# meharkhurana03/cm3d

Hardware: AMD Instinct MI355X
Metric: pseudo-label frames/sec on nuScenes-shaped sweeps (higher is better)
Workload: dtype f32; 1 GPU; c2: 256 frames/GPU x (35000x1 pts, 6 cams, 20 masks 1600x900), masks resident as rle; frames_per_gpu=256, points_per_frame=35000, masks_per_frame=20, lane_points=50000, mask_input=rle, batches_in_flight=4, distinct_batches=4, cloud_materialised=False

## Files before the change

### cm3d_amd/csrc/medoid.hip

```cpp
#include "common.h"
#include "worklist.h"
#include <stdlib.h>

#ifndef MD_WAVES
#define MD_WAVES 4
#endif
#define MD_THREADS (MD_WAVES * 64)
#ifndef MD_STAGE
#define MD_STAGE 256
#endif

#ifndef MD_LONG_MIN
#define MD_LONG_MIN 256
#endif
#ifndef MD_BATCH_LONG
#define MD_BATCH_LONG 448
#endif
#define MD_LONG_MAX 100000
static __device__ __forceinline__ bool md_two_pass(int M) { return M > MD_LONG_MIN && M < MD_LONG_MAX; }
static_assert(MD_BATCH_LONG >= MD_LONG_MIN && MD_BATCH_LONG <= CM3D_MEDOID_TILE * MD_UNI && MD_BATCH_LONG % CM3D_MEDOID_TILE == 0,
              "the batch limit is a boundary between two of the one-count classes");
static __device__ __forceinline__ bool md_batch_long(const TileDesc *desc, int ntiles) { return ntiles > 0 && __builtin_amdgcn_readfirstlane(desc[0].M) > MD_BATCH_LONG; }

#ifndef MD_APPROX_MFMA
// ... 243 lines not shown

template <typename Fetch>
static __device__ __forceinline__ void md_approx_tile(Fetch fetch, float *s_rows, int off, int M, int jt, float *__restrict__ approx_out)
{
    const int lane = cm3d_lane();
    float qx = 0.f, qy = 0.f, qz = 0.f;
    {
        const int j = jt * 64 + lane;
        const float4 q = fetch(off + min(j, M - 1));
        if (j < M) { qx = q.x; qy = q.y; qz = q.z; }
    }
    float4 g4[MDA_STAGE / 64];
#pragma unroll
    for (int c = 0; c < MDA_STAGE / 64; ++c) g4[c] = fetch(off + min(c * 64 + lane, M - 1));
    const float qn = (qx * qx + qy * qy) + qz * qz;
    const bool cols_ok = !__ballot(!mda_point_ok(qx, qy, qz, qn));
    const float bx = qx * MDA_S, by = qy * MDA_S, bz = qz * MDA_S, bn = qn * MDA_S2;
    f2 s = {0.f, 0.f};
    bool scaled = false;
    for (int i0 = 0; i0 < M; i0 += MDA_STAGE) {
        __builtin_amdgcn_wave_barrier();
        float4 rr[MDA_STAGE / 64];
        bool rows_ok = true;
#pragma unroll
        for (int c = 0; c < MDA_STAGE / 64; ++c) {
            rr[c] = make_float4(0.f, 0.f, 0.f, 0.f);
            if (i0 + c * 64 + lane < M) {
                const float4 p = g4[c];
                rr[c] = make_float4(-2.0f * p.x, -2.0f * p.y, -2.0f * p.z, (p.x * p.x + p.y * p.y) + p.z * p.z);
                rows_ok &= mda_point_ok(p.x, p.y, p.z, rr[c].w);
            }
        }
#pragma unroll
        for (int c = 0; c < MDA_STAGE / 64; ++c) g4[c] = fetch(off + min(i0 + MDA_STAGE + c * 64 + lane, M - 1));
        const bool scaled_now = MD_SCALED_ROUTES && cols_ok && !__ballot(!rows_ok);
#pragma unroll
        for (int c = 0; c < MDA_STAGE / 64; ++c) {
            float4 r = rr[c];
            if (scaled_now) r = make_float4(r.x * MDA_S, r.y * MDA_S, r.z * MDA_S, r.w * MDA_S2);
            *reinterpret_cast<float4 *>(s_rows + 4 * (c * 64 + lane)) = r;
        }
        scaled = scaled_now;
        __builtin_amdgcn_fence(__ATOMIC_RELEASE, "wavefront");
        __builtin_amdgcn_wave_barrier();
        __builtin_amdgcn_fence(__ATOMIC_ACQUIRE, "wavefront");
        const int cnt = min(MDA_STAGE, M - i0), full = cnt & ~31;
        const float a5 = full + (lane & 31) < cnt ? 1.0f : 0.0f;
        if (scaled) {
            for (int r0 = 0; r0 < full; r0 += 32) s = md_approx_step<true>(s_rows, r0, 1.0f, bx, by, bz, bn, s);
            if (cnt & 31) s = md_approx_step<true>(s_rows, full, a5, bx, by, bz, bn, s);
        } else {
            const float ux = bx * 65536.0f, uy = by * 65536.0f, uz = bz * 65536.0f, un = bn * 4294967296.0f;
            for (int r0 = 0; r0 < full; r0 += 32) s = md_approx_step<false>(s_rows, r0, 1.0f, ux, uy, uz, un, s);
            if (cnt & 31) s = md_approx_step<false>(s_rows, full, a5, ux, uy, uz, un, s);
        }
    }
    const float t0 = (s.x + __shfl_xor(s.x, 32, 64)) * 65536.0f, t1 = (s.y + __shfl_xor(s.y, 32, 64)) * 65536.0f;
    if (lane < 32) {
        const int j = jt * 64 + lane;
        if (j < M) approx_out[off + j] = t0;
        if (j + 32 < M) approx_out[off + j + 32] = t1;
    }
}

#ifndef MD_INW_MAX
#define MD_INW_MAX MD_STAGE
#endif
#ifndef MD_INW_GC
#define MD_INW_GC 2
#endif
static_assert(MD_INW_MAX <= MD_STAGE && MD_INW_GC % 2 == 0 && MD_INW_GC * 64 * sizeof(float) <= 64 * sizeof(float4),
              "a round's terms fit the storage of its 64 staged rows");

static __device__ __forceinline__ f2 md_exact_dist2s(float m2x, float m2y, float m2z, float n, float4 qa, float4 qb)
{
    f2 acc = (f2){m2x, m2x} * (f2){qa.x, qb.x};
    acc = PK_FMA(((f2){m2y, m2y}), ((f2){qa.y, qb.y}), acc);
    acc = PK_FMA(((f2){m2z, m2z}), ((f2){qa.z, qb.z}), acc);
    acc = acc + (f2){n, n};
    acc = md_pk_add_clamp01(acc, (f2){qa.w, qb.w});
    return md_sqrt_core2z(acc);
}

static __device__ __forceinline__ bool md_inwave_tile(float4 *s_row, int cnt, int M, int jt, bool act, float qx, float qy, float qz, float qn,
                                                      float &bs, int &bj)
{
    const int lane = cm3d_lane();
    const float a = md_rows<false, true, true, true>(s_row, cnt, qx, qy, qz, qn, 0.0f) * 65536.0f;
    const float rel = 1.05f * (float)(M + 2) * 1.1920928955078125e-07f, abs_e = (float)M * 2.1e-14f;
    const float e = fmaf(a, rel, abs_e);
    const float thr = cm3d_wave_reduce_t(act ? a + e : INFINITY, [](float x, float y) { return fminf(x, y); });
    const bool all = __ballot(act && !(a < INFINITY)) != 0;
    const uint64_t cm = __ballot(act && (all || !(a - e > thr)));
    const int C = (int)__popcll(cm);
    if (C < 1 || C > MD_INW_GC) return false;
    float4 q[MD_INW_GC];
    int myj = 0x7FFFFFFF;
    {
        uint64_t rest = cm;
        const int first = __builtin_ctzll(cm);
#pragma unroll
        for (int c = 0; c < MD_INW_GC; ++c) {
            const int cl = rest ? __builtin_ctzll(rest) : first;
            if (rest && lane == c) myj = jt * 64 + cl;
            rest &= rest - 1;
            q[c] = make_float4(__int_as_float(__builtin_amdgcn_readlane(__float_as_int(qx), cl)), __int_as_float(__builtin_amdgcn_readlane(__float_as_int(qy), cl)),
                               __int_as_float(__builtin_amdgcn_readlane(__float_as_int(qz), cl)), __int_as_float(__builtin_amdgcn_readlane(__float_as_int(qn), cl)));
        }
    }
    float s = 0.0f;
    for (int r0 = 0; r0 < M; r0 += 64) {
        const bool valid = r0 + lane < M;
        const int row = min(r0 + lane, cnt - 1);
        const float *f = reinterpret_cast<const float *>(s_row) + (row >> 1) * 8 + (row & 1);
        const float m2x = f[0], m2y = f[2], m2z = f[4], n = f[6];
        float *t = reinterpret_cast<float *>(s_row + r0);
        __builtin_amdgcn_fence(__ATOMIC_RELEASE, "wavefront");
        __builtin_amdgcn_wave_barrier();
        __builtin_amdgcn_fence(__ATOMIC_ACQUIRE, "wavefront");
#pragma unroll
        for (int c = 0; c < MD_INW_GC; c += 2) {
            if (c < C) {
                const f2 d = md_exact_dist2s(m2x, m2y, m2z, n, q[c], q[c + 1]);
                t[c * 64 + lane] = valid ? d.x : 0.0f;
                t[(c + 1) * 64 + lane] = valid ? d.y : 0.0f;
            }
        }
        __builtin_amdgcn_fence(__ATOMIC_RELEASE, "wavefront");
        __builtin_amdgcn_wave_barrier();
        __builtin_amdgcn_fence(__ATOMIC_ACQUIRE, "wavefront");
        if (lane < C) {
            const float4 *tr = reinterpret_cast<const float4 *>(t + lane * 64);
            const int n16 = (min(64, M - r0) + 15) >> 4;
            for (int k0 = 0; k0 < n16; ++k0) {
                float4 v[4];
#pragma unroll
                for (int k = 0; k < 4; ++k) v[k] = tr[4 * k0 + k];
#pragma unroll
                for (int k = 0; k < 4; ++k) { s = s + v[k].x; s = s + v[k].y; s = s + v[k].z; s = s + v[k].w; }
            }
        }
    }
    bs = lane < C ? s * 65536.0f : INFINITY;
    bj = myj;
    return true;
}

template <bool WITH_LONG, bool INDEXED>
__global__ __launch_bounds__(MD_THREADS, 4) void k_medoid_tiles(const float4 *__restrict__ points,
                                                              const int32_t *__restrict__ pt_off,
                                                              const int32_t *__restrict__ mask_frame, int n_masks,
                                                              const int32_t *__restrict__ tile_off,
                                                              const int32_t *__restrict__ hit_row,
                                                              const TileDesc *__restrict__ desc,
                                                              TileBest *__restrict__ tile_best, int tile_cap,
                                                              float *__restrict__ colsum_opt, float *__restrict__ approx_opt,
                                                              int32_t *__restrict__ long_list, int32_t *__restrict__ feedback)
{
    __shared__ float4 s_row_all[MD_WAVES][MD_STAGE];
    if (!WITH_LONG && blockIdx.x == 0 && threadIdx.x == 0) {
        long_list[0] = 0;
        if (feedback) feedback[0] = md_batch_long(desc, min(tile_off[n_masks], tile_cap)) ? 1 : 0;
    }
    const int wave = threadIdx.x >> 6, lane = cm3d_lane();
    float4 *s_row = s_row_all[wave];
    const int ntiles = min(tile_off[n_masks], tile_cap);
    if (ntiles <= 0) return;
    if ((approx_opt != nullptr && md_batch_long(desc, ntiles)) != WITH_LONG) return;
    for (int t = blockIdx.x * MD_WAVES + wave; t < ntiles; t += gridDim.x * MD_WAVES) {
        const TileDesc d = desc[t];
        const int off = __builtin_amdgcn_readfirstlane(d.off), M = __builtin_amdgcn_readfirstlane(d.M);
        const int jt = __builtin_amdgcn_readfirstlane(d.jt);
        const float4 *P = INDEXED ? points + pt_off[mask_frame[__builtin_amdgcn_readfirstlane(d.m)]] : points;
        auto fetch = [&](int q) { return INDEXED ? P[hit_row[q]] : P[q]; };
        const int j = jt * 64 + lane;
        const bool act = j < M;
        float qx = 0.f, qy = 0.f, qz = 0.f, qn = 0.f;
        {
            const float4 q = fetch(off + min(j, M - 1));
            if (act) {
                qx = q.x; qy = q.y; qz = q.z;
                qn = (q.x * q.x + q.y * q.y) + q.z * q.z;
            }
        }
        float s = 0.f;
        const bool col_safe = !__ballot(act && !md_col_safe(qn));
        const bool col_scal = !__ballot(act && !mda_point_ok(qx, qy, qz, qn));
        const bool direct = M <= 25;
        const bool inw_ok = !WITH_LONG && colsum_opt == nullptr && !direct && M <= MD_INW_MAX;
        bool inw = false;
        float bs_inw = INFINITY;
        int bj_inw = 0x7FFFFFFF;
        const bool approx = WITH_LONG && md_two_pass(M);
        if (WITH_LONG && approx && MD_APPROX_MFMA) {
            md_approx_tile(fetch, reinterpret_cast<float *>(s_row), off, M, jt, approx_opt);
            continue;
        }
        for (int i0 = 0; i0 < M; i0 += MD_STAGE) {
            __builtin_amdgcn_wave_barrier();
            float4 g[MD_STAGE / 64];
            bool rows_safe = true, rows_scal = true;
#pragma unroll
            for (int c = 0; c < MD_STAGE / 64; ++c)
                g[c] = fetch(off + min(i0 + c * 64 + lane, M - 1));
#pragma unroll
            for (int c = 0; c < MD_STAGE / 64; ++c) {
                if (i0 + c * 64 + lane < M) {
                    float4 r = g[c];
                    r.w = (r.x * r.x + r.y * r.y) + r.z * r.z;
                    rows_safe &= md_row_safe(r.w);
                    rows_scal &= mda_point_ok(r.x, r.y, r.z, r.w);
                    if (!direct) { r.x = -2.0f * r.x; r.y = -2.0f * r.y; r.z = -2.0f * r.z; }
                    g[c] = r;
                }
            }
            const bool scaled = MD_SCALED_ROUTES && !direct && !approx && col_scal && !__ballot(!rows_scal);
#pragma unroll
            for (int c = 0; c < MD_STAGE / 64; ++c) {
                if (i0 + c * 64 + lane < M) {
                    float4 r = g[c];
                    if (scaled) r = make_float4(r.x * MDA_S, r.y * MDA_S, r.z * MDA_S, r.w * MDA_S2);
                    md_stage(s_row, c * 64 + lane, r);
                }
            }
            int cnt = min(MD_STAGE, M - i0);
            if (!direct) {
                const int pad = (8 - (cnt & 7)) & 7;
                if (lane < pad) md_stage(s_row, cnt + lane, make_float4(0.0f, 0.0f, 0.0f, -INFINITY));
                cnt += pad;
            }
            __builtin_amdgcn_fence(__ATOMIC_RELEASE, "wavefront");
            __builtin_amdgcn_wave_barrier();
            __builtin_amdgcn_fence(__ATOMIC_ACQUIRE, "wavefront");
            const bool safe = col_safe && !__ballot(!rows_safe);
            if (scaled && inw_ok && safe && md_inwave_tile(s_row, cnt, M, jt, act, qx * MDA_S, qy * MDA_S, qz * MDA_S, qn * MDA_S2, bs_inw, bj_inw))
                inw = true;
            else if (scaled)
                s = md_rows<false, false, true, true>(s_row, cnt, qx * MDA_S, qy * MDA_S, qz * MDA_S, qn * MDA_S2, s * MDA_S) * 65536.0f;
            else
                s = direct ? md_rows<true>(s_row, cnt, qx, qy, qz, qn, s)
                           : (approx ? md_rows<false, true>(s_row, cnt, qx, qy, qz, qn, s)
                                     : (safe ? md_rows<false, false, true>(s_row, cnt, qx, qy, qz, qn, s)
                                             : (WITH_LONG ? md_rows<false>(s_row, cnt, qx, qy, qz, qn, s) : md_rows_plain(s_row, min(MD_STAGE, M - i0), qx, qy, qz, qn, s))));
        }
        if (approx) {
            if (act) approx_opt[off + j] = s;
            continue;
        }
        if (act && colsum_opt) colsum_opt[off + j] = s;
        float bs = inw ? bs_inw : (act ? s : INFINITY);
        int bj = inw ? bj_inw : (act ? j : 0x7FFFFFFF);
        auto better = [](float s1, int j1, float s2, int j2) {
            const bool n1 = s1 != s1, n2 = s2 != s2;
            if (n1 != n2) return n1;
            if (!n1 && s1 != s2) return s1 < s2;
            return j1 < j2;
        };
        {
            const Cm3dValIdx red = cm3d_wave_reduce_t(Cm3dValIdx{bs, bj}, [&](Cm3dValIdx a_, Cm3dValIdx b_) { return better(b_.s, b_.j, a_.s, a_.j) ? b_ : a_; });
            bs = red.s; bj = red.j;
        }
        if (lane == 0) { tile_best[d.t].s = bs; tile_best[d.t].j = bj; }
    }
}

__global__ __launch_bounds__(256) void k_medoid_reduce(const float4 *__restrict__ points, const int32_t *__restrict__ pt_off,
                                                       const int32_t *__restrict__ mask_frame, int n_masks,
                                                       const int32_t *__restrict__ hit_off,
                                                       const int32_t *__restrict__ tile_off,
                                                       const int32_t *__restrict__ hit_row, int idx_cap,
                                                       const TileBest *__restrict__ tile_best, int tile_cap, int two_pass,
                                                       const TileDesc *__restrict__ desc, int32_t *__restrict__ long_list,
                                                       int32_t *__restrict__ medoid_pos, float *__restrict__ centroid)
{
    const int m = blockIdx.x * blockDim.x + threadIdx.x;
    const bool is_long = two_pass && md_batch_long(desc, min(tile_off[n_masks], tile_cap)) && m < n_masks && md_two_pass(hit_off[m + 1] - hit_off[m]);
    {
        const uint64_t lm = __ballot(is_long);
        if (lm) {
            int base = 0;
            if (cm3d_lane() == 0) base = atomicAdd(&long_list[0], (int)__popcll(lm));
            base = __builtin_amdgcn_readfirstlane(base);
            if (is_long) long_list[1 + base + cm3d_mbcnt(lm)] = m;
        }
    }
    if (m >= n_masks || is_long) return;
    const int t0 = tile_off[m], t1 = min(tile_off[m + 1], tile_cap);
    int bj = -1;
    float bs = 0.f;
    for (int tb = t0; tb < t1; tb += 8) {
        TileBest bb[8];
#pragma unroll
        for (int u = 0; u < 8; ++u) bb[u] = tile_best[min(tb + u, t1 - 1)];
#pragma unroll
        for (int u = 0; u < 8; ++u) {
            const TileBest b = bb[u];
            if (tb + u >= t1 || b.j == 0x7FFFFFFF) continue;
            const bool bn = b.s != b.s, cn = bs != bs;
            if (bj < 0 || (bn && !cn) || (!bn && !cn && b.s < bs)) { bs = b.s; bj = b.j; }
        }
    }
    medoid_pos[m] = bj;
    float cx = 0.f, cy = 0.f, cz = 0.f;
    if (bj >= 0 && hit_off[m] + bj < idx_cap) {
        const float4 p = hit_row ? points[pt_off[mask_frame[m]] + hit_row[hit_off[m] + bj]] : points[hit_off[m] + bj];
        cx = p.x; cy = p.y; cz = p.z;
    }
    centroid[3 * m + 0] = cx; centroid[3 * m + 1] = cy; centroid[3 * m + 2] = cz;
}

#define MDL_WAVES 4
#define MDL_MAXC 64
#define MDL_GC 16
#define MDL_AU 16
#define MDL_TS 68

struct MdlLds {
    union {
        float t[MDL_GC][MDL_TS];
        float4 row[MD_STAGE];
    } u;
    float4 q[MDL_GC];
    int list[MDL_MAXC];
    int cand[64];
};
static_assert(sizeof(float) * MDL_GC * MDL_TS >= sizeof(float4) * MD_STAGE, "the staged rows of the column loop live in the transposition buffer");

// ... 108 lines not shown
                            s = s + v.x; s = s + v.y; s = s + v.z; s = s + v.w;
                        }
                    }
                    wave_sync();
                    p = p1; p1 = pn;
                }
                const float bs = lane < Cg ? s : INFINITY;
                const int bj = lane < Cg ? L.list[g0 + lane] : 0x7FFFFFFF;
                const Cm3dValIdx red = cm3d_wave_reduce_t(Cm3dValIdx{bs, bj}, [&](Cm3dValIdx a_, Cm3dValIdx b_) { return better(b_.s, b_.j, a_.s, a_.j) ? b_ : a_; });
                if (red.j != 0x7FFFFFFF && (best_j == 0x7FFFFFFF || better(red.s, red.j, best_s, best_j))) { best_s = red.s; best_j = red.j; }
            }
        } else {
            float4 *s_row = L.u.row;
            int *s_cand = L.cand;
            int nc = 0;
            for (int j0 = 0; j0 < M + 64; j0 += 64) {
                const int j = j0 + lane;
                bool cand = false;
                if (j < M) {
                    const double a = (double)A[j];
                    cand = all || (a - (a * rel + abs_e) <= thr);
                }
                const uint64_t cm = __ballot(cand);
                const int add = (int)__popcll(cm);
                const bool last = j0 >= M;
                if (nc + add > 64 || (last && nc > 0)) {
                    wave_sync();
                    const bool act = lane < nc;
                    const int cj = act ? s_cand[lane] : 0;
                    float qx = 0.f, qy = 0.f, qz = 0.f, qn = 0.f;
                    {
                        const float4 q = fetch(off + cj);
                        if (act) {
                            qx = q.x; qy = q.y; qz = q.z;
                            qn = (q.x * q.x + q.y * q.y) + q.z * q.z;
                        }
                    }
                    float s = 0.f;
                    for (int i0 = 0; i0 < M; i0 += MD_STAGE) {
                        __builtin_amdgcn_wave_barrier();
                        float4 g[MD_STAGE / 64];
#pragma unroll
                        for (int c = 0; c < MD_STAGE / 64; ++c)
                            g[c] = fetch(off + min(i0 + c * 64 + lane, M - 1));
#pragma unroll
                        for (int c = 0; c < MD_STAGE / 64; ++c) {
                            if (i0 + c * 64 + lane < M) {
                                float4 r = g[c];
                                r.w = (r.x * r.x + r.y * r.y) + r.z * r.z;
                                r.x = -2.0f * r.x; r.y = -2.0f * r.y; r.z = -2.0f * r.z;
                                md_stage(s_row, c * 64 + lane, r);
                            }
                        }
                        wave_sync();
                        s = md_rows<false>(s_row, min(MD_STAGE, M - i0), qx, qy, qz, qn, s);
                    }
                    const float bs = act ? s : INFINITY;
                    const int bj = act ? cj : 0x7FFFFFFF;
                    const Cm3dValIdx red = cm3d_wave_reduce_t(Cm3dValIdx{bs, bj}, [&](Cm3dValIdx a_, Cm3dValIdx b_) { return better(b_.s, b_.j, a_.s, a_.j) ? b_ : a_; });
                    if (red.j != 0x7FFFFFFF && (best_j == 0x7FFFFFFF || better(red.s, red.j, best_s, best_j))) { best_s = red.s; best_j = red.j; }
                    nc = 0;
                    __builtin_amdgcn_wave_barrier();
                }
                if (cand) s_cand[nc + cm3d_mbcnt(cm)] = j;
                nc += add;
            }
        }
        if (lane == 0) {
            int bj = best_j == 0x7FFFFFFF ? -1 : best_j;
            medoid_pos[m] = bj;
            float cx = 0.f, cy = 0.f, cz = 0.f;
            if (bj >= 0) {
                const float4 p = fetch(off + bj);
                cx = p.x; cy = p.y; cz = p.z;
            }
            centroid[3 * m + 0] = cx; centroid[3 * m + 1] = cy; centroid[3 * m + 2] = cz;
        }
    }
}

extern "C" int64_t cm3d_tile_work_bytes(int32_t n_masks, int32_t idx_cap)
{
    if (n_masks <= 0 || idx_cap <= 0) return 0;
    return md_tile_cap(n_masks, idx_cap) * (int64_t)sizeof(TileDesc);
}

extern "C" int64_t cm3d_medoid_workspace_bytes(int32_t n_masks, int32_t idx_cap)
{
    if (n_masks <= 0 || idx_cap <= 0) return 0;
    return md_tile_cap(n_masks, idx_cap) * (int64_t)(sizeof(TileBest) + sizeof(TileDesc)) + (int64_t)idx_cap * (int64_t)sizeof(float) +
           ((int64_t)n_masks + 4) * (int64_t)sizeof(int32_t);
}

extern "C" int cm3d_medoid(const float *points, const int32_t *pt_off, const int32_t *mask_frame, int32_t n_masks,
                           const int32_t *hit_off, const int32_t *tile_off, const int32_t *hit_row, int32_t idx_cap,
                           const int32_t *tile_work, int32_t *medoid_pos, float *centroid, float *colsum_opt, void *workspace,
                           int64_t workspace_bytes, cm3d_stream_t stream)
{
    return cm3d_medoid2(points, pt_off, mask_frame, n_masks, hit_off, tile_off, hit_row, idx_cap, tile_work, medoid_pos, centroid, colsum_opt,
                        workspace, workspace_bytes, 0, nullptr, stream);
}

extern "C" int cm3d_medoid2(const float *points, const int32_t *pt_off, const int32_t *mask_frame, int32_t n_masks,
                            const int32_t *hit_off, const int32_t *tile_off, const int32_t *hit_row, int32_t idx_cap,
                            const int32_t *tile_work, int32_t *medoid_pos, float *centroid, float *colsum_opt, void *workspace,
                            int64_t workspace_bytes, int32_t flags, int32_t *feedback, cm3d_stream_t stream)
{
    if (!points || !hit_off || !tile_off || !medoid_pos || !centroid || !workspace) return CM3D_ERR_ARG;
    if (hit_row && (!pt_off || !mask_frame)) return CM3D_ERR_ARG;
    if (n_masks <= 0 || idx_cap <= 0) return CM3D_ERR_ARG;
    if (workspace_bytes < cm3d_medoid_workspace_bytes(n_masks, idx_cap)) return CM3D_ERR_WORKSPACE;
    hipStream_t st = (hipStream_t)stream;
    const int64_t tile_cap64 = md_tile_cap(n_masks, idx_cap);
    const int tile_cap = (int)(tile_cap64 > 0x7FFFFFFF ? 0x7FFFFFFF : tile_cap64);
    TileDesc *own = (TileDesc *)workspace;
    TileBest *best = (TileBest *)(own + tile_cap);
    float *approx = (!colsum_opt && !(flags & 1)) ? (float *)(best + tile_cap) : nullptr;
    int32_t *long_list = (int32_t *)((float *)(best + tile_cap) + idx_cap);
    const TileDesc *desc = (const TileDesc *)tile_work;
    if (!desc) {
        hipLaunchKernelGGL(k_medoid_desc, dim3(1), dim3(1024), 0, st, n_masks, hit_off, tile_off, idx_cap, tile_cap, own);
        CM3D_CHECK_LAUNCH();
        desc = own;
    }
    int grid = (tile_cap + MD_WAVES - 1) / MD_WAVES;
    const int gmax = n_masks / 2 < 1024 ? 1024 : (n_masks / 2 > 4096 ? 4096 : n_masks / 2);
    if (grid > gmax) grid = gmax;
    auto tiles_light = hit_row ? k_medoid_tiles<false, true> : k_medoid_tiles<false, false>;
    auto tiles_heavy = hit_row ? k_medoid_tiles<true, true> : k_medoid_tiles<true, false>;
    auto second_pass = hit_row ? k_medoid_long<true> : k_medoid_long<false>;
    hipLaunchKernelGGL(tiles_light, dim3(grid), dim3(MD_THREADS), 0, st, (const float4 *)points, pt_off, mask_frame, n_masks,
                       tile_off, hit_row, desc, best, tile_cap, colsum_opt, approx, long_list, feedback);
    CM3D_CHECK_LAUNCH();
    if (approx) {
        hipLaunchKernelGGL(tiles_heavy, dim3(grid), dim3(MD_THREADS), 0, st, (const float4 *)points, pt_off, mask_frame, n_masks,
                           tile_off, hit_row, desc, best, tile_cap, colsum_opt, approx, long_list, feedback);
        CM3D_CHECK_LAUNCH();
    }
    hipLaunchKernelGGL(k_medoid_reduce, dim3((n_masks + 255) / 256), dim3(256), 0, st, (const float4 *)points, pt_off, mask_frame,
                       n_masks, hit_off, tile_off, hit_row, idx_cap, best, tile_cap, approx ? 1 : 0, desc, long_list, medoid_pos, centroid);
    CM3D_CHECK_LAUNCH();
    if (approx) {
        hipLaunchKernelGGL(second_pass, dim3(n_masks < 1024 ? n_masks : 1024), dim3(64 * MDL_WAVES), 0, st, (const float4 *)points, pt_off, mask_frame, n_masks, hit_off,
                           hit_row, idx_cap, approx, long_list, medoid_pos, centroid);
        CM3D_CHECK_LAUNCH();
    }
    return CM3D_OK;
}

__global__ __launch_bounds__(256) void k_selftest_sqrt(uint32_t first_bits, uint32_t last_bits, unsigned long long *n_bad,
                                                        uint32_t *first_bad)
{
    unsigned long long bad = 0;
    const unsigned long long span = (unsigned long long)last_bits - first_bits + 1ull;
    for (unsigned long long i = (unsigned long long)blockIdx.x * blockDim.x + threadIdx.x; i < span;
         i += (unsigned long long)gridDim.x * blockDim.x) {
        const uint32_t b = first_bits + (uint32_t)i;
        const float x = __uint_as_float(b);
        if (!md_sqrt_ok(x)) continue;
        const float want = sqrtf(x);
        const float a = md_sqrt_core2((f2){x, x}).x, c = md_sqrt_core2_ref((f2){x, x}).y, z = md_sqrt_core2z((f2){0.0f, x}).y;
        const uint32_t z0 = __float_as_uint(md_sqrt_core2z((f2){0.0f, x}).x);
        if (__float_as_uint(a) != __float_as_uint(want) || __float_as_uint(c) != __float_as_uint(want) ||
            __float_as_uint(z) != __float_as_uint(want) || z0 != 0u) {
            ++bad;
            atomicMin(first_bad, b);
        }
    }
    if (bad) atomicAdd(n_bad, bad);
}

extern "C" int cm3d_selftest_sqrt(uint32_t first_bits, uint32_t last_bits, uint64_t *n_bad, uint32_t *first_bad, cm3d_stream_t stream)
{
    if (!n_bad || !first_bad || last_bits < first_bits || (last_bits >> 31)) return CM3D_ERR_ARG;
    hipStream_t st = (hipStream_t)stream;
    if (hipMemsetAsync(n_bad, 0, sizeof(uint64_t), st) != hipSuccess) return CM3D_ERR_LAUNCH;
    if (hipMemsetAsync(first_bad, 0xFF, sizeof(uint32_t), st) != hipSuccess) return CM3D_ERR_LAUNCH;
    hipLaunchKernelGGL(k_selftest_sqrt, dim3(8192), dim3(256), 0, st, first_bits, last_bits, (unsigned long long *)n_bad, first_bad);
    CM3D_CHECK_LAUNCH();
    return CM3D_OK;
}

__global__ __launch_bounds__(64) void k_selftest_mfma(uint64_t seed, int tiles_per_wave, unsigned long long *n_bad)
{
    const int lane = cm3d_lane();
    const bool lo = lane < 32;
    uint64_t x = seed ^ (0x9E3779B97F4A7C15ull * ((uint64_t)blockIdx.x * 64 + lane + 1));
    auto next = [&]() { x ^= x << 13; x ^= x >> 7; x ^= x << 17; return x; };
    auto coord = [&](float centre, float spread) { return centre + spread * ((float)(next() & 0xFFFFFF) * (1.0f / 8388608.0f) - 1.0f); };
    unsigned long long bad = 0;
    for (int t = 0; t < tiles_per_wave; ++t) {
        const float mags[6] = {1.0f, 0.01f, 2.5f, 6.0f, 1.0f, 20.0f};
        const float mag = mags[t % 6];
        const float cx = mag * (300.0f + 40.0f * (float)(t % 37)), cy = mag * (900.0f + 25.0f * (float)(t % 53)), spread = (t & 1) ? 3.0f : 40.0f;
        const float rx = coord(cx, spread), ry = coord(cy, spread), rz = coord(1.0f, 2.0f);
        const float qx = coord(cx, spread), qy = coord(cy, spread), qz = coord(1.0f, 2.0f);
        const float rn = (rx * rx + ry * ry) + rz * rz, qn = (qx * qx + qy * qy) + qz * qz;
        const float Rx = __shfl(rx, lane & 31, 64), Ry = __shfl(ry, lane & 31, 64), Rz = __shfl(rz, lane & 31, 64), Rn = __shfl(rn, lane & 31, 64);
        const float Qx = __shfl(qx, lane & 31, 64), Qy = __shfl(qy, lane & 31, 64), Qz = __shfl(qz, lane & 31, 64), Qn = __shfl(qn, lane & 31, 64);
        f16v c = {0.f, 0.f, 0.f, 0.f, 0.f, 0.f, 0.f, 0.f, 0.f, 0.f, 0.f, 0.f, 0.f, 0.f, 0.f, 0.f};
        c = __builtin_amdgcn_mfma_f32_32x32x2f32(lo ? -2.0f * Rx : -2.0f * Ry, lo ? Qx : Qy, c, 0, 0, 0);
        c = __builtin_amdgcn_mfma_f32_32x32x2f32(lo ? -2.0f * Rz : Rn, lo ? Qz : 1.0f, c, 0, 0, 0);
        c = __builtin_amdgcn_mfma_f32_32x32x2f32(lo ? 1.0f : 0.0f, lo ? Qn : 0.0f, c, 0, 0, 0);
        f32v c2;
#pragma unroll
        for (int q = 0; q < 32; ++q) c2[q] = 0.0f;
        c2 = __builtin_amdgcn_mfma_f32_32x32x1f32(-2.0f * Rx, qx, c2, 0, 0, 0);
        c2 = __builtin_amdgcn_mfma_f32_32x32x1f32(-2.0f * Ry, qy, c2, 0, 0, 0);
        c2 = __builtin_amdgcn_mfma_f32_32x32x1f32(-2.0f * Rz, qz, c2, 0, 0, 0);
        c2 = __builtin_amdgcn_mfma_f32_32x32x1f32(Rn, 1.0f, c2, 0, 0, 0);
        c2 = __builtin_amdgcn_mfma_f32_32x32x1f32(1.0f, qn, c2, 0, 0, 0);
#pragma unroll
        for (int q = 0; q < 16; ++q) {
            const int row = (q & 3) + 8 * (q >> 2) + 4 * (lane >> 5);
            const float ix = __shfl(rx, row, 64), iy = __shfl(ry, row, 64), iz = __shfl(rz, row, 64), in_ = __shfl(rn, row, 64);
            float acc = (-2.0f * ix) * Qx;
            acc = fmaf(-2.0f * iy, Qy, acc);
            acc = fmaf(-2.0f * iz, Qz, acc);
            acc = fmaf(in_, 1.0f, acc);
// ... 40 lines not shown
```

### cm3d_amd/csrc/worklist.h

```cpp
#pragma once
#include "common.h"

struct TileDesc { int m, off, M, jt, t; };

#define MD_UNI 7
#define MD_CLASSES 16
#define MD_DESC_PER 8

static __device__ __forceinline__ int md_class(int nt)
{
    if (nt <= MD_UNI) return nt - 1;
    return MD_UNI + (nt >= 10) + (nt >= 13) + (nt >= 17) + (nt >= 22) + (nt >= 29) + (nt >= 38) + (nt >= 50) + (nt >= 66);
}

static __device__ __forceinline__ void md_class_sums(int nt, int &acc)
{
    const int lane = cm3d_lane();
#pragma unroll
    for (int c = 0; c < MD_UNI; ++c) {
        const int x = (int)__popcll(__ballot(nt == c + 1)) * (c + 1);
        acc += lane == c ? x : 0;
    }
    if (__ballot(nt > MD_UNI)) {
        const int cls = nt > MD_UNI ? md_class(nt) : -1;
#pragma unroll
        for (int c = MD_UNI; c < MD_CLASSES; ++c) {
            if (!__ballot(cls == c)) continue;
            const int x = __builtin_amdgcn_readfirstlane(cm3d_wave_sum(cls == c ? nt : 0));
            acc += lane == c ? x : 0;
        }
    }
}

static inline int64_t md_tile_cap(int32_t n_masks, int32_t idx_cap)
{
    return (int64_t)n_masks + (int64_t)idx_cap / CM3D_MEDOID_TILE + 1;
}

template <int NT, int PER = MD_DESC_PER>
static __device__ __forceinline__ void md_build_worklist(int n_masks, const int32_t *__restrict__ hit_off,
                                                         const int32_t *__restrict__ tile_off, int idx_cap, int tile_cap,
                                                         TileDesc *__restrict__ desc, int *s_hist, int *s_cur, int part = 0,
                                                         int nparts = 1)
{
    const int lane = cm3d_lane();
    if (threadIdx.x < MD_CLASSES) { s_hist[threadIdx.x] = 0; s_cur[threadIdx.x] = 0; }
    __syncthreads();
    const int nslots = (n_masks + NT - 1) / NT;
    const int per_part = (nslots + nparts - 1) / nparts;
    const int slot0 = part * per_part, slot1 = min(nslots, slot0 + per_part);
    auto tiles_of = [&](int m) {
        if (m >= n_masks) return 0;
        const int a = tile_off[m];
        return max(0, min(tile_off[m + 1], tile_cap) - a);
    };
    int wrest = 0, wbefore = 0, wmine = 0;
    for (int g0 = 0; g0 < nslots; g0 += PER) {
        int nt[PER];
#pragma unroll
        for (int q = 0; q < PER; ++q) nt[q] = tiles_of((g0 + q) * NT + (int)threadIdx.x);
#pragma unroll
        for (int q = 0; q < PER; ++q) {
            const int g = g0 + q;
            if (g >= nslots) continue;
            if (g < slot0) md_class_sums(nt[q], wbefore);
            else if (g < slot1) md_class_sums(nt[q], wmine);
            else md_class_sums(nt[q], wrest);
        }
    }
    if (lane < MD_CLASSES) {
        const int all = wrest + wbefore + wmine;
        if (all) atomicAdd(&s_hist[lane], all);
        if (wbefore) atomicAdd(&s_cur[lane], wbefore);
    }
    __syncthreads();
    if (threadIdx.x == 0) {
        int run = 0;
        for (int c = MD_CLASSES - 1; c >= 0; --c) { const int n = s_hist[c]; s_cur[c] += run; run += n; }
    }
    __syncthreads();
    int vbase = 0;
    if (lane < MD_CLASSES && wmine) vbase = atomicAdd(&s_cur[lane], wmine);
    for (int g0 = slot0; g0 < slot1; g0 += PER) {
        int t0[PER], nt[PER], off[PER], M[PER];
#pragma unroll
        for (int q = 0; q < PER; ++q) {
            const int m = (g0 + q) * NT + (int)threadIdx.x;
            t0[q] = 0; nt[q] = 0; off[q] = 0; M[q] = 0;
            if (g0 + q < slot1 && m < n_masks) {
                t0[q] = tile_off[m];
                nt[q] = tile_off[m + 1];
                off[q] = hit_off[m];
                M[q] = hit_off[m + 1];
            }
        }
#pragma unroll
        for (int q = 0; q < PER; ++q) {
            nt[q] = max(0, min(nt[q], tile_cap) - t0[q]);
            M[q] -= off[q];
            if (off[q] + M[q] > idx_cap) M[q] = max(0, idx_cap - off[q]);
        }
#pragma unroll
        for (int q = 0; q < PER; ++q) {
            if (g0 + q >= slot1) continue;
            int pos = 0;
#pragma unroll
            for (int c = 0; c < MD_UNI; ++c) {
                const uint64_t mk = __ballot(nt[q] == c + 1);
                if (!mk) continue;
                if (nt[q] == c + 1) pos = __builtin_amdgcn_readlane(vbase, c) + cm3d_mbcnt(mk) * (c + 1);
                vbase += lane == c ? (int)__popcll(mk) * (c + 1) : 0;
            }
            if (__ballot(nt[q] > MD_UNI)) {
                const int cls = nt[q] > MD_UNI ? md_class(nt[q]) : -1;
#pragma unroll
                for (int c = MD_UNI; c < MD_CLASSES; ++c) {
                    if (!__ballot(cls == c)) continue;
                    const int v = cls == c ? nt[q] : 0;
                    const int inc = cm3d_wave_incl_scan(v);
                    if (v) pos = __builtin_amdgcn_readlane(vbase, c) + inc - v;
                    vbase += lane == c ? __builtin_amdgcn_readlane(inc, 63) : 0;
                }
            }
            if (nt[q] <= 0) continue;
            const int m = (g0 + q) * NT + (int)threadIdx.x;
            for (int jt = 0; jt < nt[q]; ++jt) desc[pos + jt] = TileDesc{m, off[q], M[q], jt, t0[q] + jt};
        }
    }
}


#define MD_FROM_COUNTS_LDS(NT) (2 * MD_CLASSES + 2 * ((NT) / 64) + 8)
template <int NT>
static __device__ __forceinline__ void md_build_from_counts(int n_masks, const int32_t *__restrict__ hit_count, int idx_cap, int tile_cap,
                                                            int32_t *__restrict__ hit_off, int32_t *__restrict__ tile_off,
                                                            TileDesc *__restrict__ desc, int32_t *__restrict__ status, int *s_i,
                                                            int part, int nparts)
{
    constexpr int NW = NT / 64;
    int *s_hist = s_i, *s_cur = s_i + MD_CLASSES, *s_wc = s_i + 2 * MD_CLASSES, *s_wt = s_wc + NW, *s_tot = s_wt + NW;
    unsigned long long *s_tot64 = reinterpret_cast<unsigned long long *>(s_tot + 4);
    const int lane = cm3d_lane(), wave = (int)threadIdx.x >> 6;
    if (threadIdx.x < MD_CLASSES) { s_hist[threadIdx.x] = 0; s_cur[threadIdx.x] = 0; }
    if (threadIdx.x < 8) s_tot[threadIdx.x] = 0;
    __syncthreads();
    const int nslots = (n_masks + NT - 1) / NT;
    const int per_part = (nslots + nparts - 1) / nparts;
    const int slot0 = min(nslots, part * per_part), slot1 = min(nslots, slot0 + per_part);
    int wrest = 0, wbefore = 0, wmine = 0;
    long long cnt_before = 0, cnt_all = 0;
    int nt_before = 0, nt_all = 0;
    constexpr int PER = 4;
    for (int g0 = 0; g0 < nslots; g0 += PER) {
        int cv[PER];
#pragma unroll
        for (int q = 0; q < PER; ++q) {
            const int m = (g0 + q) * NT + (int)threadIdx.x;
            cv[q] = (g0 + q < nslots && m < n_masks) ? hit_count[m] : 0;
        }
#pragma unroll
        for (int q = 0; q < PER; ++q) {
            const int g = g0 + q;
            if (g >= nslots) continue;
            const int nt = (cv[q] + CM3D_MEDOID_TILE - 1) / CM3D_MEDOID_TILE;
            cnt_all += cv[q]; nt_all += nt;
            if (g < slot0) { md_class_sums(nt, wbefore); cnt_before += cv[q]; nt_before += nt; }
            else if (g < slot1) md_class_sums(nt, wmine);
            else md_class_sums(nt, wrest);
        }
    }
    if (lane < MD_CLASSES) {
        const int all = wrest + wbefore + wmine;
        if (all) atomicAdd(&s_hist[lane], all);
        if (wbefore) atomicAdd(&s_cur[lane], wbefore);
    }
    {
        long long cb = cnt_before, ca = cnt_all;
#pragma unroll
        for (int o = 32; o > 0; o >>= 1) { cb += __shfl_xor(cb, o, 64); ca += __shfl_xor(ca, o, 64); }
        const int tb = cm3d_wave_sum(nt_before), ta = cm3d_wave_sum(nt_all);
        if (lane == 0) {
            atomicAdd(&s_tot64[0], (unsigned long long)cb); atomicAdd(&s_tot64[1], (unsigned long long)ca);
            atomicAdd(&s_tot[2], tb); atomicAdd(&s_tot[3], ta);
        }
    }
    __syncthreads();
    const long long total64 = (long long)s_tot64[1];
    const int base_cnt = (int)(s_tot64[0] > 0x7FFFFFFFull ? 0x7FFFFFFFull : s_tot64[0]);
    const int total_cnt = (int)(total64 > 0x7FFFFFFFll ? 0x7FFFFFFFll : total64), base_nt = s_tot[2], total_nt = s_tot[3];
    const bool overflow = total64 > (long long)idx_cap || total_nt > tile_cap || total_nt < 0;
    if (threadIdx.x == 0) {
        int run = 0;
        for (int c = MD_CLASSES - 1; c >= 0; --c) { const int n = s_hist[c]; s_cur[c] += run; run += n; }
        if (part == 0) {
            hit_off[n_masks] = total_cnt;
            tile_off[n_masks] = overflow ? 0 : total_nt;
            status[2] = total_cnt;
            status[3] = total_nt;
            if (overflow) atomicOr(&status[0], 2);
        }
    }
    __syncthreads();
    int vbase = 0;
    if (lane < MD_CLASSES && wmine) vbase = atomicAdd(&s_cur[lane], wmine);
    int carry_cnt = base_cnt, carry_nt = base_nt;
    for (int g = slot0; g < slot1; ++g) {
        const int m = g * NT + (int)threadIdx.x;
        const int M = m < n_masks ? hit_count[m] : 0;
        const int nt = (M + CM3D_MEDOID_TILE - 1) / CM3D_MEDOID_TILE;
        const int ic = cm3d_wave_incl_scan(M), it = cm3d_wave_incl_scan(nt);
        __syncthreads();
        if (lane == 63) { s_wc[wave] = ic; s_wt[wave] = it; }
        __syncthreads();
        int wb_c = 0, wb_t = 0, tot_c = 0, tot_t = 0;
#pragma unroll
        for (int w = 0; w < NW; ++w) { const int a = s_wc[w], b = s_wt[w]; if (w < wave) { wb_c += a; wb_t += b; } tot_c += a; tot_t += b; }
        const int off = carry_cnt + wb_c + ic - M, t0 = carry_nt + wb_t + it - nt;
        carry_cnt += tot_c; carry_nt += tot_t;
        if (m < n_masks) { hit_off[m] = off; tile_off[m] = overflow ? 0 : t0; }
        const int ntl = (overflow || !desc) ? 0 : nt;
        int pos = 0;
#pragma unroll
        for (int c = 0; c < MD_UNI; ++c) {
            const uint64_t mk = __ballot(nt == c + 1);
            if (!mk) continue;
            if (nt == c + 1) pos = __builtin_amdgcn_readlane(vbase, c) + cm3d_mbcnt(mk) * (c + 1);
            vbase += lane == c ? (int)__popcll(mk) * (c + 1) : 0;
        }
        if (__ballot(nt > MD_UNI)) {
            const int cls = nt > MD_UNI ? md_class(nt) : -1;
#pragma unroll
            for (int c = MD_UNI; c < MD_CLASSES; ++c) {
                if (!__ballot(cls == c)) continue;
                const int v = cls == c ? nt : 0;
                const int inc = cm3d_wave_incl_scan(v);
                if (v) pos = __builtin_amdgcn_readlane(vbase, c) + inc - v;
                vbase += lane == c ? __builtin_amdgcn_readlane(inc, 63) : 0;
            }
        }
        for (int jt = 0; jt < ntl; ++jt) desc[pos + jt] = TileDesc{m, off, M, jt, t0 + jt};
    }
}
```

Measured before the change: 2.503 million frames/s.

## Align mid-size mask tiles to block quads and share pruning thresholds across waves

The worklist builder now pads the 3-tile class to four slots with hole entries and aligns the 1–4 tile classes to 4-slot boundaries. This lets all waves of a block work on tiles of the same mask, and a header entry records the shared range. Within that range, waves exchange their in-wave pruning threshold and all-infinite flag through shared memory behind a block barrier, so each tile prunes candidates with the tightest bound seen by any wave of the same mask. The aim is to send more tiles down the cheap in-wave exact path. The cost is extra workspace, hole slots that leave waves idle, and a __syncthreads per round in the light kernel.

```diff
diff --git a/cm3d_amd/csrc/medoid.hip b/cm3d_amd/csrc/medoid.hip
--- a/cm3d_amd/csrc/medoid.hip
+++ b/cm3d_amd/csrc/medoid.hip
@@ -349,18 +349,30 @@
     return md_sqrt_core2z(acc);
 }
 
-static __device__ __forceinline__ bool md_inwave_tile(float4 *s_row, int cnt, int M, int jt, bool act, float qx, float qy, float qz, float qn,
-                                                      float &bs, int &bj)
+struct MdShare { int m; float thr; int all; };
+
+static __device__ __forceinline__ void md_inwave_sums(const float4 *s_row, int cnt, int M, bool act, float qx, float qy, float qz, float qn,
+                                                      float &a, float &e, float &thr, bool &all)
+{
+    a = md_rows<false, true, true, true>(s_row, cnt, qx, qy, qz, qn, 0.0f) * 65536.0f;
+    const float rel = 1.05f * (float)(M + 2) * 1.1920928955078125e-07f, abs_e = (float)M * 2.1e-14f;
+    e = fmaf(a, rel, abs_e);
+    thr = cm3d_wave_reduce_t(act ? a + e : INFINITY, [](float x, float y) { return fminf(x, y); });
+    all = __ballot(act && !(a < INFINITY)) != 0;
+}
+
+static __device__ __forceinline__ bool md_inwave_settle(float4 *s_row, int cnt, int M, int jt, bool act, float qx, float qy, float qz, float qn,
+                                                        float a, float e, float thr, bool all, float &bs, int &bj)
 {
     const int lane = cm3d_lane();
-    const float a = md_rows<false, true, true, true>(s_row, cnt, qx, qy, qz, qn, 0.0f) * 65536.0f;
-    const float rel = 1.05f * (float)(M + 2) * 1.1920928955078125e-07f, abs_e = (float)M * 2.1e-14f;
-    const float e = fmaf(a, rel, abs_e);
-    const float thr = cm3d_wave_reduce_t(act ? a + e : INFINITY, [](float x, float y) { return fminf(x, y); });
-    const bool all = __ballot(act && !(a < INFINITY)) != 0;
     const uint64_t cm = __ballot(act && (all || !(a - e > thr)));
     const int C = (int)__popcll(cm);
-    if (C < 1 || C > MD_INW_GC) return false;
+    if (C > MD_INW_GC) return false;
+    if (C < 1) {
+        bs = INFINITY;
+        bj = 0x7FFFFFFF;
+        return true;
+    }
     float4 q[MD_INW_GC];
     int myj = 0x7FFFFFFF;
     {
@@ -419,31 +431,42 @@
                                                               const int32_t *__restrict__ mask_frame, int n_masks,
                                                               const int32_t *__restrict__ tile_off,
                                                               const int32_t *__restrict__ hit_row,
-                                                              const TileDesc *__restrict__ desc,
+                                                              const TileDesc *__restrict__ work,
                                                               TileBest *__restrict__ tile_best, int tile_cap,
                                                               float *__restrict__ colsum_opt, float *__restrict__ approx_opt,
                                                               int32_t *__restrict__ long_list, int32_t *__restrict__ feedback)
 {
     __shared__ float4 s_row_all[MD_WAVES][MD_STAGE];
+    __shared__ MdShare s_share[2][MD_WAVES];
+    const TileDesc *desc = md_work_pos(work);
     if (!WITH_LONG && blockIdx.x == 0 && threadIdx.x == 0) {
         long_list[0] = 0;
         if (feedback) feedback[0] = md_batch_long(desc, min(tile_off[n_masks], tile_cap)) ? 1 : 0;
     }
-    const int wave = threadIdx.x >> 6, lane = cm3d_lane();
+    const int wave = WITH_LONG ? (int)(threadIdx.x >> 6) : __builtin_amdgcn_readfirstlane((int)(threadIdx.x >> 6)), lane = cm3d_lane();
     float4 *s_row = s_row_all[wave];
     const int ntiles = min(tile_off[n_masks], tile_cap);
     if (ntiles <= 0) return;
     if ((approx_opt != nullptr && md_batch_long(desc, ntiles)) != WITH_LONG) return;
-    for (int t = blockIdx.x * MD_WAVES + wave; t < ntiles; t += gridDim.x * MD_WAVES) {
-        const TileDesc d = desc[t];
-        const int off = __builtin_amdgcn_readfirstlane(d.off), M = __builtin_amdgcn_readfirstlane(d.M);
+    const int npos = __builtin_amdgcn_readfirstlane(work[0].m);
+    const int sh_lo = __builtin_amdgcn_readfirstlane(work[0].off), sh_hi = __builtin_amdgcn_readfirstlane(work[0].M);
+    int turn = 0;
+    for (int tb = blockIdx.x * MD_WAVES + (WITH_LONG ? wave : 0); tb < npos; tb += gridDim.x * MD_WAVES, turn ^= 1) {
+        const int t = WITH_LONG ? tb : tb + wave;
+        const bool sharing = !WITH_LONG && tb >= sh_lo && tb < sh_hi;
+        const bool have = WITH_LONG || t < npos;
+        const TileDesc d = desc[have ? t : 0];
+        const int off = __builtin_amdgcn_readfirstlane(d.off), M = have ? __builtin_amdgcn_readfirstlane(d.M) : 0;
         const int jt = __builtin_amdgcn_readfirstlane(d.jt);
-        const float4 *P = INDEXED ? points + pt_off[mask_frame[__builtin_amdgcn_readfirstlane(d.m)]] : points;
+        if (WITH_LONG && M == 0) continue;
+        const bool live = WITH_LONG || M > 0;
+        const int dm = live ? __builtin_amdgcn_readfirstlane(d.m) : 0;
+        const float4 *P = INDEXED ? points + pt_off[mask_frame[dm]] : points;
         auto fetch = [&](int q) { return INDEXED ? P[hit_row[q]] : P[q]; };
         const int j = jt * 64 + lane;
         const bool act = j < M;
         float qx = 0.f, qy = 0.f, qz = 0.f, qn = 0.f;
-        {
+        if (live) {
             const float4 q = fetch(off + min(j, M - 1));
             if (act) {
                 qx = q.x; qy = q.y; qz = q.z;
@@ -463,7 +486,10 @@
             md_approx_tile(fetch, reinterpret_cast<float *>(s_row), off, M, jt, approx_opt);
             continue;
         }
-        for (int i0 = 0; i0 < M; i0 += MD_STAGE) {
+        for (int i0 = 0; (!WITH_LONG && i0 == 0) || i0 < M; i0 += MD_STAGE) {
+          bool scaled = false, safe = false;
+          int cnt = 0;
+          if (live) {
             __builtin_amdgcn_wave_barrier();
             float4 g[MD_STAGE / 64];
             bool rows_safe = true, rows_scal = true;
@@ -481,7 +507,7 @@
                     g[c] = r;
                 }
             }
-            const bool scaled = MD_SCALED_ROUTES && !direct && !approx && col_scal && !__ballot(!rows_scal);
+            scaled = MD_SCALED_ROUTES && !direct && !approx && col_scal && !__ballot(!rows_scal);
 #pragma unroll
             for (int c = 0; c < MD_STAGE / 64; ++c) {
                 if (i0 + c * 64 + lane < M) {
@@ -490,7 +516,7 @@
                     md_stage(s_row, c * 64 + lane, r);
                 }
             }
-            int cnt = min(MD_STAGE, M - i0);
+            cnt = min(MD_STAGE, M - i0);
             if (!direct) {
                 const int pad = (8 - (cnt & 7)) & 7;
                 if (lane < pad) md_stage(s_row, cnt + lane, make_float4(0.0f, 0.0f, 0.0f, -INFINITY));
@@ -499,8 +525,27 @@
             __builtin_amdgcn_fence(__ATOMIC_RELEASE, "wavefront");
             __builtin_amdgcn_wave_barrier();
             __builtin_amdgcn_fence(__ATOMIC_ACQUIRE, "wavefront");
-            const bool safe = col_safe && !__ballot(!rows_safe);
-            if (scaled && inw_ok && safe && md_inwave_tile(s_row, cnt, M, jt, act, qx * MDA_S, qy * MDA_S, qz * MDA_S, qn * MDA_S2, bs_inw, bj_inw))
+            safe = col_safe && !__ballot(!rows_safe);
+          }
+          bool route = false, all_inw = false;
+          float a_inw = 0.0f, e_inw = 0.0f, thr_inw = INFINITY;
+          if (!WITH_LONG && i0 == 0) {
+            route = live && scaled && inw_ok && safe;
+            if (route) md_inwave_sums(s_row, cnt, M, act, qx * MDA_S, qy * MDA_S, qz * MDA_S, qn * MDA_S2, a_inw, e_inw, thr_inw, all_inw);
+            if (sharing) {
+              if (lane == 0) s_share[turn][wave] = MdShare{route ? dm : -1, thr_inw, all_inw ? 1 : 0};
+              __syncthreads();
+            }
+            if (sharing && route) {
+#pragma unroll
+                for (int w = 0; w < MD_WAVES; ++w) {
+                    const MdShare o = s_share[turn][w];
+                    if (o.m == dm) { thr_inw = fminf(thr_inw, o.thr); all_inw = all_inw || o.all != 0; }
+                }
+            }
+          }
+          if (live) {
+            if (route && md_inwave_settle(s_row, cnt, M, jt, act, qx * MDA_S, qy * MDA_S, qz * MDA_S, qn * MDA_S2, a_inw, e_inw, thr_inw, all_inw, bs_inw, bj_inw))
                 inw = true;
             else if (scaled)
                 s = md_rows<false, false, true, true>(s_row, cnt, qx * MDA_S, qy * MDA_S, qz * MDA_S, qn * MDA_S2, s * MDA_S) * 65536.0f;
@@ -509,7 +554,9 @@
                            : (approx ? md_rows<false, true>(s_row, cnt, qx, qy, qz, qn, s)
                                      : (safe ? md_rows<false, false, true>(s_row, cnt, qx, qy, qz, qn, s)
                                              : (WITH_LONG ? md_rows<false>(s_row, cnt, qx, qy, qz, qn, s) : md_rows_plain(s_row, min(MD_STAGE, M - i0), qx, qy, qz, qn, s))));
-        }
+          }
+        }
+        if (!live) continue;
         if (approx) {
             if (act) approx_opt[off + j] = s;
             continue;
@@ -784,14 +831,14 @@
 extern "C" int64_t cm3d_tile_work_bytes(int32_t n_masks, int32_t idx_cap)
 {
     if (n_masks <= 0 || idx_cap <= 0) return 0;
-    return md_tile_cap(n_masks, idx_cap) * (int64_t)sizeof(TileDesc);
+    return md_work_cap(n_masks, idx_cap) * (int64_t)sizeof(TileDesc);
 }
 
 extern "C" int64_t cm3d_medoid_workspace_bytes(int32_t n_masks, int32_t idx_cap)
 {
     if (n_masks <= 0 || idx_cap <= 0) return 0;
-    return md_tile_cap(n_masks, idx_cap) * (int64_t)(sizeof(TileBest) + sizeof(TileDesc)) + (int64_t)idx_cap * (int64_t)sizeof(float) +
-           ((int64_t)n_masks + 4) * (int64_t)sizeof(int32_t);
+    return md_tile_cap(n_masks, idx_cap) * (int64_t)sizeof(TileBest) + md_work_cap(n_masks, idx_cap) * (int64_t)sizeof(TileDesc) +
+           (int64_t)idx_cap * (int64_t)sizeof(float) + ((int64_t)n_masks + 4) * (int64_t)sizeof(int32_t);
 }
 
 extern "C" int cm3d_medoid(const float *points, const int32_t *pt_off, const int32_t *mask_frame, int32_t n_masks,
@@ -816,15 +863,16 @@
     const int64_t tile_cap64 = md_tile_cap(n_masks, idx_cap);
     const int tile_cap = (int)(tile_cap64 > 0x7FFFFFFF ? 0x7FFFFFFF : tile_cap64);
     TileDesc *own = (TileDesc *)workspace;
-    TileBest *best = (TileBest *)(own + tile_cap);
+    TileBest *best = (TileBest *)(own + md_work_cap(n_masks, idx_cap));
     float *approx = (!colsum_opt && !(flags & 1)) ? (float *)(best + tile_cap) : nullptr;
     int32_t *long_list = (int32_t *)((float *)(best + tile_cap) + idx_cap);
-    const TileDesc *desc = (const TileDesc *)tile_work;
-    if (!desc) {
+    const TileDesc *work = (const TileDesc *)tile_work;
+    if (!work) {
         hipLaunchKernelGGL(k_medoid_desc, dim3(1), dim3(1024), 0, st, n_masks, hit_off, tile_off, idx_cap, tile_cap, own);
         CM3D_CHECK_LAUNCH();
-        desc = own;
-    }
+        work = own;
+    }
+    const TileDesc *desc = md_work_pos(work);
     int grid = (tile_cap + MD_WAVES - 1) / MD_WAVES;
     const int gmax = n_masks / 2 < 1024 ? 1024 : (n_masks / 2 > 4096 ? 4096 : n_masks / 2);
     if (grid > gmax) grid = gmax;
@@ -832,11 +880,11 @@
     auto tiles_heavy = hit_row ? k_medoid_tiles<true, true> : k_medoid_tiles<true, false>;
     auto second_pass = hit_row ? k_medoid_long<true> : k_medoid_long<false>;
     hipLaunchKernelGGL(tiles_light, dim3(grid), dim3(MD_THREADS), 0, st, (const float4 *)points, pt_off, mask_frame, n_masks,
-                       tile_off, hit_row, desc, best, tile_cap, colsum_opt, approx, long_list, feedback);
+                       tile_off, hit_row, work, best, tile_cap, colsum_opt, approx, long_list, feedback);
     CM3D_CHECK_LAUNCH();
     if (approx) {
         hipLaunchKernelGGL(tiles_heavy, dim3(grid), dim3(MD_THREADS), 0, st, (const float4 *)points, pt_off, mask_frame, n_masks,
-                           tile_off, hit_row, desc, best, tile_cap, colsum_opt, approx, long_list, feedback);
+                           tile_off, hit_row, work, best, tile_cap, colsum_opt, approx, long_list, feedback);
         CM3D_CHECK_LAUNCH();
     }
     hipLaunchKernelGGL(k_medoid_reduce, dim3((n_masks + 255) / 256), dim3(256), 0, st, (const float4 *)points, pt_off, mask_frame,
diff --git a/cm3d_amd/csrc/worklist.h b/cm3d_amd/csrc/worklist.h
--- a/cm3d_amd/csrc/worklist.h
+++ b/cm3d_amd/csrc/worklist.h
@@ -2,6 +2,7 @@
 #include "common.h"
 
 struct TileDesc { int m, off, M, jt, t; };
+#define MD_HOLE (TileDesc{-1, 0, 0, 0, -1})
 
 #define MD_UNI 7
 #define MD_CLASSES 16
@@ -13,12 +14,14 @@
     return MD_UNI + (nt >= 10) + (nt >= 13) + (nt >= 17) + (nt >= 22) + (nt >= 29) + (nt >= 38) + (nt >= 50) + (nt >= 66);
 }
 
+static __device__ __forceinline__ constexpr int md_class_slots(int c) { return c == 2 ? 4 : c + 1; }
+
 static __device__ __forceinline__ void md_class_sums(int nt, int &acc)
 {
     const int lane = cm3d_lane();
 #pragma unroll
     for (int c = 0; c < MD_UNI; ++c) {
-        const int x = (int)__popcll(__ballot(nt == c + 1)) * (c + 1);
+        const int x = (int)__popcll(__ballot(nt == c + 1)) * md_class_slots(c);
         acc += lane == c ? x : 0;
     }
     if (__ballot(nt > MD_UNI)) {
@@ -32,18 +35,48 @@
     }
 }
 
-static inline int64_t md_tile_cap(int32_t n_masks, int32_t idx_cap)
+static __host__ __device__ inline int64_t md_tile_cap(int32_t n_masks, int32_t idx_cap)
 {
     return (int64_t)n_masks + (int64_t)idx_cap / CM3D_MEDOID_TILE + 1;
+}
+static __host__ __device__ inline int64_t md_work_cap(int32_t n_masks, int32_t idx_cap)
+{
+    return md_tile_cap(n_masks, idx_cap) + (int64_t)idx_cap / (2 * CM3D_MEDOID_TILE) + 16;
+}
+static __host__ __device__ inline int md_pos_cap(int32_t n_masks, int32_t idx_cap)
+{
+    const int64_t c = md_work_cap(n_masks, idx_cap) - 1;
+    return (int)(c > 0x7FFFFFFF ? 0x7FFFFFFF : c);
+}
+static __host__ __device__ __forceinline__ const TileDesc *md_work_pos(const TileDesc *work) { return work + 1; }
+static __device__ __forceinline__ TileDesc md_class_starts(const int *s_hist, int *s_cur, TileDesc *pos, int pos_cap)
+{
+    const bool mid = (s_hist[3] | s_hist[2] | s_hist[1]) != 0;
+    int run = 0, lo = 0, hi = 0;
+    for (int c = MD_CLASSES - 1; c >= 0; --c) {
+        if (c == 3 && mid) {
+            for (; run & 3; ++run)
+                if (pos && run < pos_cap) pos[run] = MD_HOLE;
+            lo = run;
+        }
+        const int n = s_hist[c];
+        s_cur[c] += run;
+        run += n;
+        if (c == 1 && mid) hi = (run + 3) & ~3;
+    }
+    if (s_hist[2] && !(s_hist[1] | s_hist[0])) --run;
+    return TileDesc{min(run, pos_cap), lo, hi, 0, 0};
 }
 
 template <int NT, int PER = MD_DESC_PER>
 static __device__ __forceinline__ void md_build_worklist(int n_masks, const int32_t *__restrict__ hit_off,
                                                          const int32_t *__restrict__ tile_off, int idx_cap, int tile_cap,
-                                                         TileDesc *__restrict__ desc, int *s_hist, int *s_cur, int part = 0,
+                                                         TileDesc *__restrict__ work, int *s_hist, int *s_cur, int part = 0,
                                                          int nparts = 1)
 {
     const int lane = cm3d_lane();
+    TileDesc *const desc = work + 1;
+    const int pos_cap = md_pos_cap(n_masks, idx_cap);
     if (threadIdx.x < MD_CLASSES) { s_hist[threadIdx.x] = 0; s_cur[threadIdx.x] = 0; }
     __syncthreads();
     const int nslots = (n_masks + NT - 1) / NT;
@@ -75,8 +108,8 @@
     }
     __syncthreads();
     if (threadIdx.x == 0) {
-        int run = 0;
-        for (int c = MD_CLASSES - 1; c >= 0; --c) { const int n = s_hist[c]; s_cur[c] += run; run += n; }
+        const TileDesc head = md_class_starts(s_hist, s_cur, part == 0 ? desc : nullptr, pos_cap);
+        if (part == 0) work[0] = head;
     }
     __syncthreads();
     int vbase = 0;
@@ -108,8 +141,8 @@
             for (int c = 0; c < MD_UNI; ++c) {
                 const uint64_t mk = __ballot(nt[q] == c + 1);
                 if (!mk) continue;
-                if (nt[q] == c + 1) pos = __builtin_amdgcn_readlane(vbase, c) + cm3d_mbcnt(mk) * (c + 1);
-                vbase += lane == c ? (int)__popcll(mk) * (c + 1) : 0;
+                if (nt[q] == c + 1) pos = __builtin_amdgcn_readlane(vbase, c) + cm3d_mbcnt(mk) * md_class_slots(c);
+                vbase += lane == c ? (int)__popcll(mk) * md_class_slots(c) : 0;
             }
             if (__ballot(nt[q] > MD_UNI)) {
                 const int cls = nt[q] > MD_UNI ? md_class(nt[q]) : -1;
@@ -124,7 +157,9 @@
             }
             if (nt[q] <= 0) continue;
             const int m = (g0 + q) * NT + (int)threadIdx.x;
-            for (int jt = 0; jt < nt[q]; ++jt) desc[pos + jt] = TileDesc{m, off[q], M[q], jt, t0[q] + jt};
+            for (int jt = 0; jt < nt[q]; ++jt)
+                if (pos + jt < pos_cap) desc[pos + jt] = TileDesc{m, off[q], M[q], jt, t0[q] + jt};
+            if (nt[q] == 3 && pos + 3 < pos_cap) desc[pos + 3] = MD_HOLE;
         }
     }
 }
@@ -134,9 +169,11 @@
 template <int NT>
 static __device__ __forceinline__ void md_build_from_counts(int n_masks, const int32_t *__restrict__ hit_count, int idx_cap, int tile_cap,
                                                             int32_t *__restrict__ hit_off, int32_t *__restrict__ tile_off,
-                                                            TileDesc *__restrict__ desc, int32_t *__restrict__ status, int *s_i,
+                                                            TileDesc *__restrict__ work, int32_t *__restrict__ status, int *s_i,
                                                             int part, int nparts)
 {
+    TileDesc *const desc = work ? work + 1 : nullptr;
+    const int pos_cap = md_pos_cap(n_masks, idx_cap);
     constexpr int NW = NT / 64;
     int *s_hist = s_i, *s_cur = s_i + MD_CLASSES, *s_wc = s_i + 2 * MD_CLASSES, *s_wt = s_wc + NW, *s_tot = s_wt + NW;
     unsigned long long *s_tot64 = reinterpret_cast<unsigned long long *>(s_tot + 4);
@@ -190,9 +227,9 @@
     const int total_cnt = (int)(total64 > 0x7FFFFFFFll ? 0x7FFFFFFFll : total64), base_nt = s_tot[2], total_nt = s_tot[3];
     const bool overflow = total64 > (long long)idx_cap || total_nt > tile_cap || total_nt < 0;
     if (threadIdx.x == 0) {
-        int run = 0;
-        for (int c = MD_CLASSES - 1; c >= 0; --c) { const int n = s_hist[c]; s_cur[c] += run; run += n; }
+        const TileDesc head = md_class_starts(s_hist, s_cur, (part == 0 && !overflow) ? desc : nullptr, pos_cap);
         if (part == 0) {
+            if (work) work[0] = overflow ? TileDesc{0, 0, 0, 0, 0} : head;
             hit_off[n_masks] = total_cnt;
             tile_off[n_masks] = overflow ? 0 : total_nt;
             status[2] = total_cnt;
@@ -224,8 +261,8 @@
         for (int c = 0; c < MD_UNI; ++c) {
             const uint64_t mk = __ballot(nt == c + 1);
             if (!mk) continue;
-            if (nt == c + 1) pos = __builtin_amdgcn_readlane(vbase, c) + cm3d_mbcnt(mk) * (c + 1);
-            vbase += lane == c ? (int)__popcll(mk) * (c + 1) : 0;
+            if (nt == c + 1) pos = __builtin_amdgcn_readlane(vbase, c) + cm3d_mbcnt(mk) * md_class_slots(c);
+            vbase += lane == c ? (int)__popcll(mk) * md_class_slots(c) : 0;
         }
         if (__ballot(nt > MD_UNI)) {
             const int cls = nt > MD_UNI ? md_class(nt) : -1;
@@ -238,6 +275,8 @@
                 vbase += lane == c ? __builtin_amdgcn_readlane(inc, 63) : 0;
             }
         }
-        for (int jt = 0; jt < ntl; ++jt) desc[pos + jt] = TileDesc{m, off, M, jt, t0 + jt};
-    }
-}
+        for (int jt = 0; jt < ntl; ++jt)
+            if (pos + jt < pos_cap) desc[pos + jt] = TileDesc{m, off, M, jt, t0 + jt};
+        if (ntl == 3 && pos + 3 < pos_cap) desc[pos + 3] = MD_HOLE;
+    }
+}
```

After: 2.518 million frames/s, median of 6. About the same (+0.6%).
